# mushroomfire/mdapy

Hardware: AMD Instinct MI355X
Metric: atoms/sec for neighbor+CNA on 10M-atom FCC Cu; 1/2/4/8-GPU scaling (higher is better)
Workload: dtype f64 (CNA pair tests: f32 filter + f64 finish, labels exact); 1 GPU; FCC Cu a=3.615, 136^3 cells per GPU (10061824 atoms/GPU, 10061824 total), build_neighbor(rc=0.854a=3.08721, max_neigh=16) + fixed-cutoff CNA as one C-ABI call (mdh_build_neighbor_fcna: lists and labels), positions resident in HBM; atoms_per_gpu=10061824, max_neigh=16, parallelism=single, world_size_checked=1, launched_by=single process

## Files before the change

### mdapy_amd/csrc/cell_grid.hip

```cpp
#include "common.hpp"
#include "grid.hpp"
#include "assign_groups.hpp"
#include "grid_plan.hpp"
#include <algorithm>
#include <atomic>
#include <mutex>
#include <vector>

namespace mdh {
static std::atomic<int> g_indirect{[] { const char *e = std::getenv("MDH_INDIRECT"); return e ? std::atoi(e) : 1; }()};

struct CellPlanes { int p0, p1, p2, p3; int *bad; };
template <bool TRI, int K, bool SLOT = false>
__global__ __launch_bounds__(256) void k_assign(const double *__restrict__ x, const double *__restrict__ y,
                                                const double *__restrict__ z, int64_t N, DBox b, Grid g,
                                                int wrap_first, int2 *__restrict__ ent,
                                                unsigned *__restrict__ cell_count, unsigned *__restrict__ ctl, unsigned gen,
                                                double slack, unsigned short *__restrict__ mv, CellPlanes win,
                                                CellGrid::Packed *__restrict__ rec, int drop_absent, int *__restrict__ slots = nullptr,
                                                int2 *__restrict__ spill = nullptr, unsigned *__restrict__ spill_n = nullptr, int64_t slot_hi = 0)
{
    const int lane = threadIdx.x & 63;
    const int64_t i0 = ((int64_t)blockIdx.x * (blockDim.x >> 6) + (threadIdx.x >> 6)) * (64 * K) + lane;
    bool moved = false, outside = false, coded = false;
    double xr[K], yr[K], zr[K];
#pragma unroll
    for (int k = 0; k < K; ++k) {
        const int64_t i = i0 + 64 * k;
        xr[k] = yr[k] = zr[k] = 0.0;
        if (i < N) { xr[k] = x[i]; yr[k] = y[i]; zr[k] = z[i]; }
    }
    int cells[K];
#pragma unroll
    for (int k = 0; k < K; ++k) {
        const int64_t i = i0 + 64 * k;
        int cell = -1 - lane;
        const bool absent = drop_absent && i < N && xr[k] != xr[k];
// ... 54 lines not shown
#pragma unroll
    for (int k = 0; k < K; ++k) {
        const unsigned bs = __shfl(base[k], head[k], 64);
        const int64_t i = i0 + 64 * k;
        if (SLOT) {
            if (i < N && cells[k] >= 0) {
                const unsigned s = bs + (unsigned)slot[k];
                if (s < (unsigned)SLOT_CAP) slots[slot_pos(cells[k], (int)s, slot_hi)] = (int)i;
                else spill[atomicAdd(spill_n, 1u)] = make_int2(cells[k], (int)i);
            }
            continue;
        }
        if (i < N)
            ent[i] = make_int2(cells[k], (int)(bs + (unsigned)slot[k]));
    }
    if (__any(moved) && lane == 0)
        ctl[1] = gen;
    if (__any(coded) && lane == 0)
        ctl[2] = gen;
    if (__any(outside) && lane == 0)
        *win.bad = 1;
}

static constexpr int SCAN_BLOCK = 256;
static constexpr int SCAN_ITEMS = 4;
static constexpr int SCAN_ITEMS_BIG = 32;
static constexpr int64_t SCAN_BIG_FROM = 1 << 19;

__device__ __forceinline__ unsigned wave_incl_scan(unsigned v, int lane)
{
#pragma unroll
    for (int d = 1; d < 64; d <<= 1) {
        unsigned t = __shfl_up(v, d, 64);
        if (lane >= d) v += t;
// ... 193 lines not shown
    if (W == 4) {
        ce(0, 1); ce(2, 3); ce(0, 2); ce(1, 3); ce(1, 2);
    } else {
        ce(0, 1); ce(2, 3); ce(4, 5); ce(6, 7);
        ce(0, 2); ce(1, 3); ce(4, 6); ce(5, 7);
        ce(1, 2); ce(5, 6);
        ce(0, 4); ce(1, 5); ce(2, 6); ce(3, 7);
        ce(2, 4); ce(3, 5);
        ce(1, 2); ce(3, 4); ce(5, 6);
    }
#pragma unroll
    for (int u = 0; u < W; ++u)
        if (u < n) order[s + u] = id[u];
}

__device__ __forceinline__ void report_big_cell(unsigned *__restrict__ ctl, unsigned gen, int *__restrict__ sink, int n)
{
    if (__hip_atomic_load(&ctl[3], __ATOMIC_RELAXED, __HIP_MEMORY_SCOPE_AGENT) == gen)
        return;
    __hip_atomic_store(&ctl[3], gen, __ATOMIC_RELAXED, __HIP_MEMORY_SCOPE_AGENT);
    sink[1] = n;
}

__global__ __launch_bounds__(256) void k_sort_cells(const int *__restrict__ cell_start, int *__restrict__ order,
                                                    int64_t ncell, const int64_t *__restrict__ key, int *__restrict__ tmp,
                                                    unsigned *__restrict__ ctl = nullptr, unsigned gen = 0, int *__restrict__ big_sink = nullptr)
{
    int64_t c = (int64_t)blockIdx.x * blockDim.x + threadIdx.x;
    if (c >= ncell)
        return;
    const int s = cell_start[c], e = cell_start[c + 1];
    const int n = e - s;
    if (big_sink && n > SLOT_CAP) report_big_cell(ctl, gen, big_sink, n);
    if (n <= 1)
        return;
    if (n <= 4) {
        if (key) sort_cell_net<4, int64_t>(order, s, n, key);
        else sort_cell_net<4, int>(order, s, n, nullptr);
// ... 46 lines not shown
    if (staged) {
        for (int a = sub; a < n; a += 8) {
            const int mine = ids[lc * SORT_DENSE_CAP + a];
            int larger = 0;
            for (int q = 0; q < n; ++q) larger += ids[lc * SORT_DENSE_CAP + q] > mine ? 1 : 0;
            order[s + larger] = mine;
        }
    } else if (big) {
        for (int a = sub; a < n; a += 8) {
            const int mine = tmp[s + a];
            int larger = 0;
            for (int q = 0; q < n; ++q) larger += tmp[s + q] > mine ? 1 : 0;
            order[s + larger] = mine;
        }
    }
}

__global__ __launch_bounds__(256) void k_sort_slots(const unsigned *__restrict__ count, int *__restrict__ slots, int64_t ncell,
                                                    unsigned *__restrict__ idle, int64_t idle_n, unsigned *__restrict__ ctl, unsigned gen,
                                                    int *__restrict__ big_sink, int *__restrict__ flags, int64_t slot_hi)
{
    const int64_t c = (int64_t)blockIdx.x * blockDim.x + threadIdx.x;
    if (c == 0) {
        flags[0] = ctl[1] == gen ? 1 : 0; flags[1] = 0; flags[2] = 0; flags[3] = 0;
        flags[4] = ctl[2] == gen ? 1 : 0; flags[5] = 0; flags[6] = 0; flags[7] = 0;
    }
    if (c < idle_n) idle[c] = 0u;
    if (c >= ncell)
        return;
    const int full = (int)count[c];
    if (full > SLOT_CAP) report_big_cell(ctl, gen, big_sink, full);
    const int n = min(full, SLOT_CAP);
    if (n <= 1)
        return;
    int4 *cell = reinterpret_cast<int4 *>(slots + 4 * c), *cell_hi = reinterpret_cast<int4 *>(slots + slot_hi + 4 * c);
    auto ce = [](int &a, int &b) { const int hi = max(a, b), lo = min(a, b); a = hi; b = lo; };
    int4 q0 = cell[0];
    int id[8] = {q0.x, n > 1 ? q0.y : INT32_MIN, n > 2 ? q0.z : INT32_MIN, n > 3 ? q0.w : INT32_MIN, INT32_MIN, INT32_MIN, INT32_MIN, INT32_MIN};
    if (SLOT_CAP == 4 || n <= 4) {
        ce(id[0], id[1]); ce(id[2], id[3]); ce(id[0], id[2]); ce(id[1], id[3]); ce(id[1], id[2]);
        cell[0] = make_int4(id[0], id[1], id[2], id[3]);
        return;
    }
    const int4 q1 = cell_hi[0];
    id[4] = q1.x; id[5] = n > 5 ? q1.y : INT32_MIN; id[6] = n > 6 ? q1.z : INT32_MIN; id[7] = n > 7 ? q1.w : INT32_MIN;
    ce(id[0], id[1]); ce(id[2], id[3]); ce(id[4], id[5]); ce(id[6], id[7]);
    ce(id[0], id[2]); ce(id[1], id[3]); ce(id[4], id[6]); ce(id[5], id[7]);
    ce(id[1], id[2]); ce(id[5], id[6]);
    ce(id[0], id[4]); ce(id[1], id[5]); ce(id[2], id[6]); ce(id[3], id[7]);
    ce(id[2], id[4]); ce(id[3], id[5]);
    ce(id[1], id[2]); ce(id[3], id[4]); ce(id[5], id[6]);
    cell[0] = make_int4(id[0], id[1], id[2], id[3]);
    cell_hi[0] = make_int4(id[4], id[5], id[6], id[7]);
}

__global__ __launch_bounds__(256) void k_gather(const double *__restrict__ x, const double *__restrict__ y,
                                                const double *__restrict__ z, const int *__restrict__ order,
                                                double *__restrict__ xs, double *__restrict__ ys,
                                                double *__restrict__ zs, int64_t N,
                                                const unsigned short *__restrict__ mv, unsigned short *__restrict__ mvs,
                                                CellGrid::Packed *__restrict__ pk, const int *__restrict__ any_code,
                                                const int *__restrict__ n_binned)
{
    int64_t p = (int64_t)blockIdx.x * blockDim.x + threadIdx.x;
    if (p >= N)
        return;
    if (n_binned && p >= *n_binned)
        return;
// ... 251 lines not shown
    const size_t N = (size_t)bd.N;
    if (bd.slot()) {
        bd.slot_block = static_cast<unsigned *>(sc.alloc_kept(2 * sizeof(unsigned) * (size_t)(g.ncell + 128), Scope::KEEP_SLOT));
        if (bd.slot_block) {
            const size_t half = sc.held_bytes(bd.slot_block) / 8;
            bd.sb = slot_block_state(bd.slot_block);
            bd.cell_count = bd.slot_block + (size_t)bd.sb->next * half + 64;
            bd.slot_idle = bd.slot_block + (size_t)(1 - bd.sb->next) * half;
            bd.slot_idle_n = std::min<int64_t>(bd.sb->dirty[1 - bd.sb->next], (int64_t)half);
        }
        cg.slot_hi = 4 * g.ncell;
    } else {
        bd.cell_count = static_cast<unsigned *>(sc.alloc_kept(sizeof(unsigned) * (size_t)g.ncell, Scope::KEEP_ZERO));
    }
    bd.ctl = static_cast<unsigned *>(sc.alloc_kept(scan_ctl_bytes(g.ncell), Scope::KEEP_SCAN));
    cg.flags = sc.alloc_n<int>(8);
    cg.cell_start = bd.slot() ? reinterpret_cast<int *>(bd.cell_count) : sc.alloc_n<int>((size_t)g.ncell + 1);
    bd.ent = sc.alloc_n<int2>(N);
    cg.order = sc.alloc_n<int>(bd.slot() ? (size_t)g.ncell * SLOT_CAP + 4 : N + 4);
    bd.mv = sc.alloc_n<unsigned short>(N);
    switch (bd.pl.form) {
    case GridPlan::ARRAYS:
        cg.xs = sc.alloc_n<double>(N);
        cg.ys = sc.alloc_n<double>(N);
        cg.zs = sc.alloc_n<double>(N);
        cg.mvs = sc.alloc_n<unsigned short>(N);
        break;
    case GridPlan::RECORDS_GATHERED: cg.pk = sc.alloc_n<CellGrid::Packed>(N); break;
    case GridPlan::RECORDS_MOVED: cg.pk = sc.alloc_n<CellGrid::Packed>(N); bd.rec = sc.alloc_n<CellGrid::Packed>(N); break;
    case GridPlan::INDIRECT: case GridPlan::SLOT: break;
    }
// ... 9 lines not shown
    for (int d = 0; d < 3; ++d) nb[d] = std::max(1.0, std::floor(bd.b.thick[d] / edge));
    hipLaunchKernelGGL(k_order_far_flag, dim3(1), dim3(1024), 0, bd.st, bd.x, bd.y, bd.z, bd.N, bd.b, nb[0], nb[1], nb[2], word);
}

template <bool TRI, int K, bool SLOT>
static void launch_assign(const GridBuild &bd, const CellGrid &cg)
{
    const Grid &g = cg.g;
    const double slack = 0.01 / (g.rc_inv > 0 ? g.rc_inv : 1.0);
    const CellPlanes win{bd.pl.p0, bd.pl.p1, bd.pl.p2, bd.pl.p3, bd.bad};
    int2 *const ent = SLOT ? nullptr : bd.ent, *const spill = SLOT ? bd.ent : nullptr;
    int *const slots = SLOT ? cg.order : nullptr;
    unsigned *const spill_n = SLOT ? bd.cell_count - 64 : nullptr;
    hipLaunchKernelGGL((k_assign<TRI, K, SLOT>), dim3(grid_for(bd.N, 256 * K)), dim3(256), 0, bd.st, bd.x, bd.y, bd.z, bd.N, bd.b, g, (int)bd.rq.wrap_first,
                       ent, bd.cell_count, bd.ctl, bd.gen, slack, bd.mv, win, bd.rec, bd.pl.form != GridPlan::ARRAYS ? 1 : 0, slots, spill, spill_n,
                       SLOT ? cg.slot_hi : (int64_t)0);
}
static void bin_atoms(const GridBuild &bd, const CellGrid &cg)
{
    switch ((bd.b.tri ? 4 : 0) | (bd.pl.assign4 ? 2 : 0) | (bd.slot() ? 1 : 0)) {
    case 0: launch_assign<false, 1, false>(bd, cg); break;
    case 1: launch_assign<false, 1, true>(bd, cg); break;
    case 2: launch_assign<false, 4, false>(bd, cg); break;
    case 3: launch_assign<false, 4, true>(bd, cg); break;
    case 4: launch_assign<true, 1, false>(bd, cg); break;
    case 5: launch_assign<true, 1, true>(bd, cg); break;
    case 6: launch_assign<true, 4, false>(bd, cg); break;
    case 7: launch_assign<true, 4, true>(bd, cg); break;
    }
}

static int finish_slot_grid(Scope &sc, const GridBuild &bd, CellGrid &cg)
{
    const Grid &g = cg.g;
    hipLaunchKernelGGL(k_sort_slots, dim3(grid_for(std::max<int64_t>(g.ncell, bd.slot_idle_n), 256)), dim3(256), 0, bd.st, bd.cell_count, cg.order, g.ncell,
                       bd.slot_idle, bd.slot_idle_n, bd.ctl, bd.gen, bd.hist, cg.flags, cg.slot_hi);
    MDH_HIP(hipGetLastError());
    {
        std::lock_guard<std::mutex> lk(g_slot_mu);
        SlotBlock *sb = bd.sb;
        sb->dirty[1 - sb->next] = 0;
        sb->dirty[sb->next] = g.ncell + 64;
        sb->next = 1 - sb->next;
    }
    sc.keep_confirm(bd.slot_block);
    cg.big_stamp = bd.ctl + 3; cg.big_gen = bd.gen; cg.big_sink = bd.hist;
    cg.slot_cap = SLOT_CAP;
    cg.spill = bd.ent;
    cg.n_spill = bd.cell_count - 64;
    cg.ix = bd.x; cg.iy = bd.y; cg.iz = bd.z; cg.imv = bd.mv;
    return MDH_OK;
// ... 200 lines not shown
```

### mdapy_amd/csrc/grid.hpp

```cpp
#pragma once
#include "common.hpp"
#include "grid_plan.hpp"
#include <atomic>
#include <cmath>

namespace mdh {

struct Grid {
    int nc[3];
    int64_t ncell;
    double rc_inv;
    int mode;
};

namespace img {
constexpr int MAX_M = 14;
constexpr int ATOM_NEUTRAL = 15 | (15 << 5) | (15 << 10);
constexpr int CELL_NEUTRAL = 1 | (1 << 2) | (1 << 4);
constexpr int NEUTRAL = 16 | (16 << 5) | (16 << 10);
__host__ __device__ __forceinline__ int combine(int cc, int ca)
{
    return ((cc & 3) + (ca & 31)) | ((((cc >> 2) & 3) + ((ca >> 5) & 31)) << 5) | ((((cc >> 4) & 3) + ((ca >> 10) & 31)) << 10);
}
__host__ __device__ __forceinline__ int axis(int code, int d) { return ((code >> (5 * d)) & 31) - 16; }
// ... 8 lines not shown
    mutable bool flags_fresh = false;
    int *cell_start = nullptr;
    int *order = nullptr;
    double *xs = nullptr, *ys = nullptr, *zs = nullptr;
    int *flags = nullptr;
    unsigned short *mvs = nullptr;
    struct Packed { double x, y, z; int id, code; };
    Packed *pk = nullptr;
    const double *ix = nullptr, *iy = nullptr, *iz = nullptr;
    const unsigned short *imv = nullptr;
    int slot_cap = 0;
    int64_t slot_hi = 0;
    const int2 *spill = nullptr;
    const unsigned *n_spill = nullptr;
    int64_t n_binned = 0;
    const unsigned *big_stamp = nullptr;
    unsigned big_gen = 0;
    int *big_sink = nullptr;
};
__host__ __device__ __forceinline__ int64_t slot_pos(int64_t c, int k, int64_t hi) { return c * 4 + k + (k >= 4 ? hi - 4 : 0); }
struct SlotSpill { const int2 *list = nullptr; const unsigned *n = nullptr; int64_t hi = 0; };
struct SortedView {
    const double *xs, *ys, *zs;
    const int *order;
    const CellGrid::Packed *pk;
    bool indirect;
    __device__ __forceinline__ void get(int64_t q, double &x, double &y, double &z, int &id) const
    {
        if (pk) { const CellGrid::Packed r = pk[q]; x = r.x; y = r.y; z = r.z; id = r.id; }
        else if (indirect) { id = order[q]; x = xs[id]; y = ys[id]; z = zs[id]; }
        else { x = xs[q]; y = ys[q]; z = zs[q]; id = order[q]; }
    }
    __device__ __forceinline__ void get4(const int64_t (&q)[4], double (&x)[4], double (&y)[4], double (&z)[4], int (&id)[4]) const
    {
        if (pk) {
#pragma unroll
// ... 156 lines not shown
            for (int bb = c1 - 1; bb <= c1 + 1; ++bb) {
                const int64_t base = ((int64_t)ca * g.nc[1] + pmod(bb, g.nc[1])) * g.nc[2];
                for (int seg = 0; seg < (zrun ? 1 : 3); ++seg) {
                    const int64_t cell = base + (zrun ? c2 - 1 : pmod(c2 - 1 + seg, g.nc[2]));
                    if (SLOT) {
                        f(CellPiece{cell, cell_start[cell]});
                    } else {
                        const int s = cell_start[cell];
                        f(CellPiece{s, cell_start[cell + (zrun ? 3 : 1)] - s});
                    }
                }
            }
        }
    }
    __device__ __forceinline__ bool overflowed(const CellPiece &pc) const { return SLOT && pc.n > SLOT_CAP; }
    __device__ __forceinline__ int64_t pos(const CellPiece &pc, int k) const { return SLOT ? slot_pos(pc.at, k, sp.hi) : pc.at + k; }
    __device__ __forceinline__ int next_id_below(int64_t cell, int prev) const
    {
        int best = -1;
        for (int u = 0; u < SLOT_CAP; ++u) {
            const int v = sv.order[slot_pos(cell, u, sp.hi)];
            if (v < prev && v > best) best = v;
        }
        const unsigned ns = *sp.n;
        for (unsigned w = 0; w < ns; ++w) {
            const int2 e = sp.list[w];
            if ((int64_t)e.x == cell && e.y < prev && e.y > best) best = e.y;
        }
        return best;
    }
    template <class F>
// ... 50 lines not shown
```

### mdapy_amd/csrc/neighbor.hip

```cpp
#include "common.hpp"
#include "grid.hpp"
#include "cna_core.hpp"
#include <algorithm>

namespace mdh {

static int *g_moved_probe = nullptr;
int g_neighbor_variant = 0;

template <bool TRI, int MODE>
struct Centre {
    const DBox &b;
    int i;
    double xi, yi, zi, rcsq;
    int *__restrict__ verlet;
    double *__restrict__ dist;
    int64_t row, M;

    __device__ __forceinline__ Centre(const DBox &b_, int i_, double x, double y, double z, double rc, int *v, double *d, int64_t M_)
        : b(b_), i(i_), xi(x), yi(y), zi(z), rcsq(rc * rc), verlet(v), dist(d), row((int64_t)i_ * M_), M(M_) {}
    __device__ __forceinline__ bool hit(int j, double xq, double yq, double zq, double &d2) const
    {
        double dx = xq - xi, dy = yq - yi, dz = zq - zi;
        pbc<TRI>(b, dx, dy, dz);
// ... 11 lines not shown
    {
        if (lane == 0) nn[i] = cnt;
        if (MODE == 2) {
            const double pad = rc + 1.0;
            for (int64_t n = cnt + lane; n < M; n += stride) {
                verlet[row + n] = -1;
                dist[row + n] = pad;
            }
        }
    }
};

template <bool TRI, int MODE, bool SLOT>
__device__ __forceinline__ int overflowed_cell(const CellView<SLOT> &cv, const Centre<TRI, MODE> &c, int64_t cell, int cnt, bool store)
{
    for (int j = cv.next_id_below(cell, 0x7fffffff); j >= 0; j = cv.next_id_below(cell, j)) {
        double d2;
        if (!c.hit(j, cv.sv.xs[j], cv.sv.ys[j], cv.sv.zs[j], d2))
            continue;
        if (store) c.store(cnt, j, d2);
        ++cnt;
    }
    return cnt;
}

template <bool TRI, int MODE, bool SLOT>
__device__ __forceinline__ int neighbor_one(const CellView<SLOT> &cv, const Grid &g, const Centre<TRI, MODE> &c, double rc,
                                            int *__restrict__ nn, int c0, int c1, int c2)
{
    int cnt = 0;
    cv.for_each_piece(g, c0, c1, c2, [&](const CellPiece &pc) {
        if (cv.overflowed(pc)) {
            cnt = overflowed_cell(cv, c, pc.at, cnt, true);
            return;
        }
        for (int k0 = 0; k0 < pc.n; k0 += 4) {
            double xq[4], yq[4], zq[4], d2;
            int jq[4];
            int64_t q[4];
#pragma unroll
            for (int u = 0; u < 4; ++u) q[u] = cv.pos(pc, min(k0 + u, pc.n - 1));
            cv.sv.get4(q, xq, yq, zq, jq);
#pragma unroll
            for (int u = 0; u < 4; ++u)
                if (k0 + u < pc.n && c.hit(jq[u], xq[u], yq[u], zq[u], d2)) c.store(cnt++, jq[u], d2);
        }
    });
    c.finish(nn, rc, cnt, 0, 1);
    return cnt;
}

template <bool TRI, int MODE, bool SLOT>
__device__ __forceinline__ int neighbor_one_wave(const CellView<SLOT> &cv, const Grid &g, const Centre<TRI, MODE> &c, double rc,
                                                 int *__restrict__ nn, int c0, int c1, int c2)
{
    const int lane = (int)(threadIdx.x & 63);
    int cnt = 0;
    cv.for_each_piece(g, c0, c1, c2, [&](const CellPiece &pc) {
        if (cv.overflowed(pc)) {
            cnt = overflowed_cell(cv, c, pc.at, cnt, lane == 0);
            return;
        }
        for (int k0 = 0; k0 < pc.n; k0 += 64) {
            const int k = k0 + lane;
            bool hit = false;
            int j = -1;
            double d2 = 0.0;
            if (k < pc.n) {
                double xq, yq, zq;
                cv.sv.get(cv.pos(pc, k), xq, yq, zq, j);
                hit = c.hit(j, xq, yq, zq, d2);
            }
            const unsigned long long m = __ballot(hit);
            if (hit) c.store(cnt + __popcll(m & ((1ull << lane) - 1ull)), j, d2);
            cnt += __popcll(m);
        }
    });
    c.finish(nn, rc, cnt, lane, 64);
    return cnt;
}

template <bool TRI, int MODE, bool SLOT>
__device__ __forceinline__ void neighbor_atoms_body(const CellView<SLOT> &cv, int64_t N, const DBox &b, const Grid &g,
                                                  double rc, int *__restrict__ verlet, double *__restrict__ dist,
                                                  int *__restrict__ nn, int64_t M, int *__restrict__ max_count,
// ... 20 lines not shown
            }
        }
        if (mine) {
            cnt = max(cnt, neighbor_one(cv, g, Centre<TRI, MODE>(b, i, xi, yi, zi, rc, verlet, dist, M), rc, nn, c0, c1, c2));
            if (tf.cna_todo) defer(tf.cna_todo, i);
        }
    }
    if (MODE == 0) raise_max(max_count, wave_max(cnt));
}

template <bool TRI, int MODE, bool SLOT>
__global__ __launch_bounds__(256) void k_neighbor(SortedView sv, const int *__restrict__ cell_start, int64_t N, DBox b, Grid g, double rc,
                                                  int *__restrict__ verlet, double *__restrict__ dist, int *__restrict__ nn, int64_t M,
                                                  int *__restrict__ max_count, TileFilter tf, SlotSpill sp)
{
    if (tf.big_sink && blockIdx.x == 0 && threadIdx.x == 0)
        *tf.big_sink = *tf.big_stamp == tf.big_gen ? 1 : 0;
    neighbor_atoms_body<TRI, MODE>(CellView<SLOT>{sv, cell_start, sp}, N, b, g, rc, verlet, dist, nn, M, max_count, tf);
}

template <bool TRI, int MODE, bool SLOT>
__device__ __forceinline__ void neighbor_tiles_body(const CellView<SLOT> &cv, const DBox &b, const Grid &g, double rc,
                                                        int *__restrict__ verlet, double *__restrict__ dist, int *__restrict__ nn,
                                                        int64_t M, int *__restrict__ max_count, const TileFilter &tf)
{
    if (tf.moved && *tf.moved != 0)
        return;
    const int nlist = min(*tf.any, tf.list_cap);
    int best = 0;
    const int ncol = tf.tile * tf.tile;
    const int wave = (int)(threadIdx.x >> 6), nwave = (int)(blockDim.x >> 6);
// ... 38 lines not shown
{
    if (tf.listed_sink && blockIdx.x == 0 && threadIdx.x == 0)
        *tf.listed_sink = min(*tf.any, tf.list_cap);
    if (tf.big_sink && blockIdx.x == 0 && threadIdx.x == 0)
        *tf.big_sink = *tf.big_stamp == tf.big_gen ? 1 : 0;
    const CellView<SLOT> cv{sv, cell_start, sp};
    if (tf.moved && *tf.moved != 0) neighbor_atoms_body<TRI, MODE>(cv, N, b, g, rc, verlet, dist, nn, M, max_count, tf);
    else neighbor_tiles_body<TRI, MODE>(cv, b, g, rc, verlet, dist, nn, M, max_count, tf);
}

template <int MODE>
static void launch_neighbor(hipStream_t st, const CellGrid &cg, int64_t N, const DBox &b, double rc, int *verlet,
                            double *dist, int *nn, int64_t M, int *max_count, TileFilter tf = TileFilter{})
{
    dim3 grid(std::min(grid_for(N, 256), tf.list ? 2048 : 8192)), block(256);
    const SlotSpill sp{cg.spill, cg.n_spill, cg.slot_hi};
#define MDH_MOP(KERNEL, TRI, SLOT, ...) hipLaunchKernelGGL((KERNEL<TRI, MODE, SLOT>), grid, block, 0, st, view_of(cg), cg.cell_start, __VA_ARGS__, b, cg.g, rc, verlet, dist, nn, M, max_count, tf, sp)
    if (tf.list) {
        if (cg.slot_cap) { if (b.tri) MDH_MOP(k_neighbor_mop, true, true, N); else MDH_MOP(k_neighbor_mop, false, true, N); }
        else { if (b.tri) MDH_MOP(k_neighbor_mop, true, false, N); else MDH_MOP(k_neighbor_mop, false, false, N); }
        return;
    }
    if (cg.slot_cap) { if (b.tri) MDH_MOP(k_neighbor, true, true, N); else MDH_MOP(k_neighbor, false, true, N); }
    else { if (b.tri) MDH_MOP(k_neighbor, true, false, N); else MDH_MOP(k_neighbor, false, false, N); }
#undef MDH_MOP
}

__global__ __launch_bounds__(256) void k_max_i32(const int *__restrict__ v, int64_t n, int *__restrict__ out)
{
    int m = 0;
    for (int64_t i = (int64_t)blockIdx.x * blockDim.x + threadIdx.x; i < n; i += (int64_t)gridDim.x * blockDim.x) m = max(m, v[i]);
// ... 281 lines not shown
```

### mdapy_amd/csrc/neighbor_lane.hip

```cpp
#include "common.hpp"
#include "grid.hpp"
#include "cna_core.hpp"
#include <algorithm>
#include <cmath>
#include <type_traits>
#include <cstdio>
#include <cstdlib>
#include <cstring>

namespace mdh {
namespace lane {

constexpr int NW = 4;
constexpr int CEN_CAP = 80 * NW;
__host__ __device__ constexpr int ticket_row(int M, bool cna_rows) { return (cna_rows && ((M + 4) & ~3) < 28) ? 28 : ((M + 4) & ~3); }
static constexpr int NEUTRAL = img::CELL_NEUTRAL;
static constexpr int NEUTRAL3 = img::NEUTRAL;

struct FastDiv {
    unsigned mul, sh1, sh2, d;
    __device__ __forceinline__ unsigned div(unsigned n) const
    {
        const unsigned t = __umulhi(mul, n);
        return (t + ((n - t) >> sh1)) >> sh2;
// ... 231 lines not shown
            const int y = __builtin_amdgcn_mov_dpp(x, 0xB1, 0xF, 0xF, true);
            P[pp + 1][w] = bit_select(odd1, P[pp + 1][w], y);
            P[pp][w] = bit_select(odd1, y, P[pp][w]);
        }
#pragma unroll
    for (int pp = 0; pp < 2; ++pp)
#pragma unroll
        for (int w = 0; w < 4; ++w) {
            const int x = bit_select(odd2, P[pp][w], P[pp + 2][w]);
            const int y = __builtin_amdgcn_mov_dpp(x, 0x4E, 0xF, 0xF, true);
            P[pp + 2][w] = bit_select(odd2, P[pp + 2][w], y);
            P[pp][w] = bit_select(odd2, y, P[pp][w]);
        }
}

struct IndirectSrc { const double *x, *y, *z; const unsigned short *mv; const int *order; };
__device__ __forceinline__ CellGrid::Packed load_atom(const IndirectSrc &src, int id, int coded)
{
    int code = (int)img::ATOM_NEUTRAL;
    if (coded) code = src.mv[id];
    return CellGrid::Packed{src.x[id], src.y[id], src.z[id], id, code};
}
struct __attribute__((packed, aligned(4))) Ids4 { int v[4]; };
template <bool IND>
__device__ __forceinline__ CellGrid::Packed load_record(const CellGrid::Packed *__restrict__ pk, const IndirectSrc &src, int q, int coded)
{
    if (!IND)
        return pk[q];
    return load_atom(src, src.order[q], coded);
}

// ... 54 lines not shown
            t2 = t.id - (int)col * nt2;
            t0 = (int)ts.by_nt1.div(col);
            t1 = (int)col - t0 * nt1;
        }
        t.T0 = t0 * TXY; t.T1 = t1 * TXY; t.T2 = t2 * TZ;
        t.empty = t.T2 >= g.nc[2];
        return t;
    };
    auto halo_of = [&](const Tile &t) {
        Halo h{0, 0, NEUTRAL, 0, false, false};
        if (tid < NH && !t.empty) {
            const int hcol = (int)(((unsigned)tid * ts.mhz) >> 16);
            h.hz = tid - hcol * HZ;
            const int hx = (int)(((unsigned)hcol * ts.mhxy) >> 16), hy = hcol - hx * HXY;
            const int g0 = t.T0 + hx - 1, g1 = t.T1 + hy - 1, g2 = t.T2 + h.hz - 1;
            const bool in0 = b.pbc[0] ? (g0 >= -1 && g0 <= g.nc[0]) : (g0 >= 0 && g0 < g.nc[0]);
            const bool in1 = b.pbc[1] ? (g1 >= -1 && g1 <= g.nc[1]) : (g1 >= 0 && g1 < g.nc[1]);
            const bool in2 = b.pbc[2] ? (g2 >= -1 && g2 <= g.nc[2]) : (g2 >= 0 && g2 < g.nc[2]);
            if (in0 && in1 && in2) {
                bool over = false;
                const int a0 = g0 < 0 ? g0 + g.nc[0] : (g0 >= g.nc[0] ? g0 - g.nc[0] : g0);
                const int a1 = g1 < 0 ? g1 + g.nc[1] : (g1 >= g.nc[1] ? g1 - g.nc[1] : g1);
                const int a2 = g2 < 0 ? g2 + g.nc[2] : (g2 >= g.nc[2] ? g2 - g.nc[2] : g2);
                const int c = (a0 * g.nc[1] + a1) * g.nc[2] + a2;
                if (SLOT) {
                    const int n = cell_start[c];
                    h.src = c << 2;
                    h.cnt = min(n, SLOT_CAP);
                    over = n > SLOT_CAP;
                } else {
                    h.src = cell_start[c];
                    h.cnt = cell_start[c + 1] - h.src;
                }
                const int n0 = g0 < 0 ? 1 : (g0 >= g.nc[0] ? -1 : 0);
                const int n1 = g1 < 0 ? 1 : (g1 >= g.nc[1] ? -1 : 0);
                const int n2 = g2 < 0 ? 1 : (g2 >= g.nc[2] ? -1 : 0);
                h.img = (n0 + 1) | ((n1 + 1) << 2) | ((n2 + 1) << 4);
                if (SLOT && over) h.img |= 64;
                h.edge = (!b.pbc[0] && (a0 == 0 || a0 == g.nc[0] - 1)) || (!b.pbc[1] && (a1 == 0 || a1 == g.nc[1] - 1)) ||
                         (!b.pbc[2] && (a2 == 0 || a2 == g.nc[2] - 1));
                h.centre = hx >= 1 && hx <= TXY && hy >= 1 && hy <= TXY && h.hz >= 1 && h.hz <= TZ && g0 < g.nc[0] && g1 < g.nc[1] && g2 < g.nc[2] &&
                           g0 >= cen_lo && g0 < cen_hi;
            }
        }
        return h;
    };
    auto request = [&](const Halo &h, double (&ra)[4], double (&rb)[4], double (&rc4)[4], int (&rd)[4], int (&rm)[4]) {
        Ids4 ids{};
        if (IND) ids = *reinterpret_cast<const Ids4 *>(isrc.order + h.src);
#pragma unroll
        for (int v = 0; v < 4; ++v) {
            const int q = h.cnt > 0 ? h.src + min(v, h.cnt - 1) : 0;
            const CellGrid::Packed a = IND ? load_atom(isrc, v < h.cnt ? ids.v[v] : (h.cnt > 0 ? ids.v[0] : 0), coded) : load_record<false>(pk, isrc, q, coded);
            ra[v] = a.x; rb[v] = a.y; rc4[v] = a.z; rd[v] = a.id; rm[v] = a.code;
        }
    };
    for (int jt = jt0 + (int)(blockIdx.x >> 3); jt < per; jt += (int)(gridDim.x >> 3)) {
        const int slot = (int)(blockIdx.x & 7) * per + jt;
        if (slot >= nlive)
            break;
        const Tile tile = tile_of(slot);
        STAMP(0);
        Halo cur = halo_of(tile);
#ifdef MDH_STAMPS
        asm volatile("" : "+v"(cur.src), "+v"(cur.cnt));
        STAMP(1);
#endif
        double pa[4], pb[4], pc[4];
// ... 67 lines not shown
                            uy = (float)((bb[v] - b.h[4] * (double)img::axis(code, 1)) - Y0);
                            uz = (float)((c[v] - b.h[8] * (double)img::axis(code, 2)) - Z0);
                            general = true;
                        }
                        if (!TRI && edge)
                            far = far || !(ux >= flo && ux <= fhx && uy >= flo && uy <= fhx && uz >= flo && uz <= fhz);
                        const int p = off0 + k + v;
                        f4[p] = make_float4(ux, uy, uz, __int_as_float(d[v]));
                        lxy[p] = make_double2(a[v], bb[v]);
                        lz[p] = c[v];
                        lsh[p] = (unsigned short)code;
                        if (centre_cell) cen[coff + k + v] = (unsigned)p | ((unsigned)tid << 11);
                    }
                }
            };
            if (TK8) {
                for (int k = 0; k < cnt; k += 4) {
                    double a[4], bb[4], c[4];
                    int d[4], m[4];
#pragma unroll
                    for (int v = 0; v < 4; ++v) {
                        if (k == 0) { a[v] = pa[v]; bb[v] = pb[v]; c[v] = pc[v]; d[v] = pd[v]; m[v] = pm[v]; }
                        else {
                            const int kv = min(k + v, cnt - 1);
                            const int q = src + kv + (SLOT && kv >= 4 ? slot_hi : 0);
                            const CellGrid::Packed r = load_record<IND>(pk, isrc, q, coded);
                            a[v] = r.x; bb[v] = r.y; c[v] = r.z; d[v] = r.id; m[v] = r.code;
                        }
                    }
                    stage4(k, a, bb, c, d, m);
                }
            } else {
                double a[4], bb[4], c[4];
                int d[4], m[4];
#pragma unroll
                for (int v = 0; v < 4; ++v) { a[v] = pa[v]; bb[v] = pb[v]; c[v] = pc[v]; d[v] = pd[v]; m[v] = pm[v]; }
                for (int k = 0; k < cnt; k += 4) {
                    double na[4], nb[4], nc[4];
                    int nd[4], nm[4];
#pragma unroll
                    for (int v = 0; v < 4; ++v) {
                        const int kv = min(k + 4 + v, cnt - 1);
                        const int q = src + kv + (SLOT && kv >= 4 ? slot_hi : 0);
                        const CellGrid::Packed r = load_record<IND>(pk, isrc, q, coded);
                        na[v] = r.x; nb[v] = r.y; nc[v] = r.z; nd[v] = r.id; nm[v] = r.code;
                    }
                    stage4(k, a, bb, c, d, m);
#pragma unroll
                    for (int v = 0; v < 4; ++v) { a[v] = na[v]; bb[v] = nb[v]; c[v] = nc[v]; d[v] = nd[v]; m[v] = nm[v]; }
                }
            }
            if (general) s_flag[0] = 1;
            if (far) s_flag[1] = 1;
        }
        __syncthreads();
        STAMP(3);
        if (ok && (s_flag[1] | s_flag[2]))
            ok = false;
// ... 644 lines not shown
        hipLaunchKernelGGL(k_tile_compact, dim3(grid_for(ntiles, 256)), dim3(256), 0, st, live, slot, (int)ntiles, tile_list);
        const int64_t est_live = std::max<int64_t>(1, plan.occupied / std::max(1, ts.txy * ts.txy * ts.tz) * 2);
        per = std::max(1, std::min(per, (int)((est_live + est_live / 4 + 7) / 8)));
        list_mode = 1;
    }
    const dim3 grid((unsigned)(per * 8));
    const size_t lds = lds_bytes(plan.cap, count ? 1 : M, plan.tk8, plan.rw, pattern != nullptr);
    const int cen_lo = cg.cen_hi > cg.cen_lo ? cg.cen_lo : 0, cen_hi = cg.cen_hi > cg.cen_lo ? cg.cen_hi : 0x7fffffff;
    const int Mi = (int)M, wp = fill_pads ? (rows.ids_only ? 3 : 1) : 0;
    const float negc = -plan.mid;
    const int nt2b = nt[2] * nsub;
    const bool slice_pass = plan.last_listed != 0;
    const dim3 grid2(1024u);
    const Shape ts2 = make_shape(ts.txy, 1, nt[1], nt2b);
    const bool indirect = !cg.pk;
    const lane::IndirectSrc isrc{cg.ix, cg.iy, cg.iz, cg.imv, cg.order};
    const int slot_hi = cg.slot_cap ? (int)(cg.slot_hi - 4) : 0;
#define MDH_LANE_PASS_I(COUNT, TRI, LOOP, FCNA, TK8, IND, SLOT, GRID, JT0, ...)                                                                 \
    do {                                                                                                                                  \
        if (lds > 60 * 1024)                             \
            (void)hipFuncSetAttribute(reinterpret_cast<const void *>(&k_neighbor_lane<COUNT, TRI, LOOP, FCNA, TK8, IND, SLOT>), hipFuncAttributeMaxDynamicSharedMemorySize, (int)lds); \
        hipLaunchKernelGGL((k_neighbor_lane<COUNT, TRI, LOOP, FCNA, TK8, IND, SLOT>), GRID, dim3(NW * 64), lds, st, cg.pk, cg.cell_start, b, \
                           cg.g, rc, negc, plan.T, verlet, dist, nn, Mi, wp, plan.cap, cg.flags, nullptr, __VA_ARGS__, pattern, tf.cna_todo, JT0, plan.rw, tile_base, plan.listed_sink, \
                           cen_lo, cen_hi, isrc, slot_hi); \
    } while (0)
#define MDH_LANE_PASS(COUNT, TRI, LOOP, FCNA, TK8, GRID, JT0, ...)                                                                        \
    do {                                                                                                                                  \
        if (indirect && cg.slot_cap) MDH_LANE_PASS_I(COUNT, TRI, LOOP, FCNA, TK8, true, true, GRID, JT0, __VA_ARGS__);                    \
        else if (indirect) MDH_LANE_PASS_I(COUNT, TRI, LOOP, FCNA, TK8, true, false, GRID, JT0, __VA_ARGS__);                             \
        else MDH_LANE_PASS_I(COUNT, TRI, LOOP, FCNA, TK8, false, false, GRID, JT0, __VA_ARGS__);                                          \
    } while (0)
// ... 58 lines not shown
```

Before: 7.651 billion atoms/s.

## Drop slot-sort kernel; sort cell slots on the fly in neighbor consumers

Removes the separate k_sort_slots launch. The idle-buffer zeroing and the flag setting move into k_assign, and the per-cell sorting network moves into the neighbor kernels, which sort the slot ids in registers when they load them. Big-cell reporting is moved into the consumers as well. The halo setup also gains a fast path for interior tiles that skips the boundary wrap arithmetic. This saves one kernel launch and a full pass over the slot array, at the cost of repeating the sort each time a cell is read (27 neighbours) and adding flag-protocol complexity.

New measurement: 7.709 billion atoms/s, median of 6. No clear change (+0.8%).

```diff
diff --git a/mdapy_amd/csrc/cell_grid.hip b/mdapy_amd/csrc/cell_grid.hip
--- a/mdapy_amd/csrc/cell_grid.hip
+++ b/mdapy_amd/csrc/cell_grid.hip
@@ -18,9 +18,17 @@
                                                 unsigned *__restrict__ cell_count, unsigned *__restrict__ ctl, unsigned gen,
                                                 double slack, unsigned short *__restrict__ mv, CellPlanes win,
                                                 CellGrid::Packed *__restrict__ rec, int drop_absent, int *__restrict__ slots = nullptr,
-                                                int2 *__restrict__ spill = nullptr, unsigned *__restrict__ spill_n = nullptr, int64_t slot_hi = 0)
+                                                int2 *__restrict__ spill = nullptr, unsigned *__restrict__ spill_n = nullptr, int64_t slot_hi = 0,
+                                                unsigned *__restrict__ idle = nullptr, int64_t idle_n = 0)
 {
     const int lane = threadIdx.x & 63;
+    if (SLOT) {
+        const int64_t stride = 4 * (int64_t)gridDim.x * blockDim.x;
+        for (int64_t w = 4 * ((int64_t)blockIdx.x * blockDim.x + threadIdx.x); w < idle_n; w += stride) {
+            if (w + 4 <= idle_n) *reinterpret_cast<uint4 *>(idle + w) = make_uint4(0u, 0u, 0u, 0u);
+            else for (int64_t t = w; t < idle_n; ++t) idle[t] = 0u;
+        }
+    }
     const int64_t i0 = ((int64_t)blockIdx.x * (blockDim.x >> 6) + (threadIdx.x >> 6)) * (64 * K) + lane;
     bool moved = false, outside = false, coded = false;
     double xr[K], yr[K], zr[K];
@@ -105,10 +113,14 @@
         if (i < N)
             ent[i] = make_int2(cells[k], (int)(bs + (unsigned)slot[k]));
     }
-    if (__any(moved) && lane == 0)
+    if (__any(moved) && lane == 0) {
         ctl[1] = gen;
-    if (__any(coded) && lane == 0)
+        if (SLOT) spill_n[8] = 1u;
+    }
+    if (__any(coded) && lane == 0) {
         ctl[2] = gen;
+        if (SLOT) spill_n[8 + 4] = 1u;
+    }
     if (__any(outside) && lane == 0)
         *win.bad = 1;
 }
@@ -332,14 +344,6 @@
         if (u < n) order[s + u] = id[u];
 }
 
-__device__ __forceinline__ void report_big_cell(unsigned *__restrict__ ctl, unsigned gen, int *__restrict__ sink, int n)
-{
-    if (__hip_atomic_load(&ctl[3], __ATOMIC_RELAXED, __HIP_MEMORY_SCOPE_AGENT) == gen)
-        return;
-    __hip_atomic_store(&ctl[3], gen, __ATOMIC_RELAXED, __HIP_MEMORY_SCOPE_AGENT);
-    sink[1] = n;
-}
-
 __global__ __launch_bounds__(256) void k_sort_cells(const int *__restrict__ cell_start, int *__restrict__ order,
                                                     int64_t ncell, const int64_t *__restrict__ key, int *__restrict__ tmp,
                                                     unsigned *__restrict__ ctl = nullptr, unsigned gen = 0, int *__restrict__ big_sink = nullptr)
@@ -416,44 +420,6 @@
             order[s + larger] = mine;
         }
     }
-}
-
-__global__ __launch_bounds__(256) void k_sort_slots(const unsigned *__restrict__ count, int *__restrict__ slots, int64_t ncell,
-                                                    unsigned *__restrict__ idle, int64_t idle_n, unsigned *__restrict__ ctl, unsigned gen,
-                                                    int *__restrict__ big_sink, int *__restrict__ flags, int64_t slot_hi)
-{
-    const int64_t c = (int64_t)blockIdx.x * blockDim.x + threadIdx.x;
-    if (c == 0) {
-        flags[0] = ctl[1] == gen ? 1 : 0; flags[1] = 0; flags[2] = 0; flags[3] = 0;
-        flags[4] = ctl[2] == gen ? 1 : 0; flags[5] = 0; flags[6] = 0; flags[7] = 0;
-    }
-    if (c < idle_n) idle[c] = 0u;
-    if (c >= ncell)
-        return;
-    const int full = (int)count[c];
-    if (full > SLOT_CAP) report_big_cell(ctl, gen, big_sink, full);
-    const int n = min(full, SLOT_CAP);
-    if (n <= 1)
-        return;
-    int4 *cell = reinterpret_cast<int4 *>(slots + 4 * c), *cell_hi = reinterpret_cast<int4 *>(slots + slot_hi + 4 * c);
-    auto ce = [](int &a, int &b) { const int hi = max(a, b), lo = min(a, b); a = hi; b = lo; };
-    int4 q0 = cell[0];
-    int id[8] = {q0.x, n > 1 ? q0.y : INT32_MIN, n > 2 ? q0.z : INT32_MIN, n > 3 ? q0.w : INT32_MIN, INT32_MIN, INT32_MIN, INT32_MIN, INT32_MIN};
-    if (SLOT_CAP == 4 || n <= 4) {
-        ce(id[0], id[1]); ce(id[2], id[3]); ce(id[0], id[2]); ce(id[1], id[3]); ce(id[1], id[2]);
-        cell[0] = make_int4(id[0], id[1], id[2], id[3]);
-        return;
-    }
-    const int4 q1 = cell_hi[0];
-    id[4] = q1.x; id[5] = n > 5 ? q1.y : INT32_MIN; id[6] = n > 6 ? q1.z : INT32_MIN; id[7] = n > 7 ? q1.w : INT32_MIN;
-    ce(id[0], id[1]); ce(id[2], id[3]); ce(id[4], id[5]); ce(id[6], id[7]);
-    ce(id[0], id[2]); ce(id[1], id[3]); ce(id[4], id[6]); ce(id[5], id[7]);
-    ce(id[1], id[2]); ce(id[5], id[6]);
-    ce(id[0], id[4]); ce(id[1], id[5]); ce(id[2], id[6]); ce(id[3], id[7]);
-    ce(id[2], id[4]); ce(id[3], id[5]);
-    ce(id[1], id[2]); ce(id[3], id[4]); ce(id[5], id[6]);
-    cell[0] = make_int4(id[0], id[1], id[2], id[3]);
-    cell_hi[0] = make_int4(id[4], id[5], id[6], id[7]);
 }
 
 __global__ __launch_bounds__(256) void k_gather(const double *__restrict__ x, const double *__restrict__ y,
@@ -735,7 +701,7 @@
         bd.cell_count = static_cast<unsigned *>(sc.alloc_kept(sizeof(unsigned) * (size_t)g.ncell, Scope::KEEP_ZERO));
     }
     bd.ctl = static_cast<unsigned *>(sc.alloc_kept(scan_ctl_bytes(g.ncell), Scope::KEEP_SCAN));
-    cg.flags = sc.alloc_n<int>(8);
+    cg.flags = bd.slot() ? (bd.slot_block ? reinterpret_cast<int *>(bd.cell_count - 64 + 8) : nullptr) : sc.alloc_n<int>(8);
     cg.cell_start = bd.slot() ? reinterpret_cast<int *>(bd.cell_count) : sc.alloc_n<int>((size_t)g.ncell + 1);
     bd.ent = sc.alloc_n<int2>(N);
     cg.order = sc.alloc_n<int>(bd.slot() ? (size_t)g.ncell * SLOT_CAP + 4 : N + 4);
@@ -775,7 +741,7 @@
     unsigned *const spill_n = SLOT ? bd.cell_count - 64 : nullptr;
     hipLaunchKernelGGL((k_assign<TRI, K, SLOT>), dim3(grid_for(bd.N, 256 * K)), dim3(256), 0, bd.st, bd.x, bd.y, bd.z, bd.N, bd.b, g, (int)bd.rq.wrap_first,
                        ent, bd.cell_count, bd.ctl, bd.gen, slack, bd.mv, win, bd.rec, bd.pl.form != GridPlan::ARRAYS ? 1 : 0, slots, spill, spill_n,
-                       SLOT ? cg.slot_hi : (int64_t)0);
+                       SLOT ? cg.slot_hi : (int64_t)0, SLOT ? bd.slot_idle : nullptr, SLOT ? bd.slot_idle_n : (int64_t)0);
 }
 static void bin_atoms(const GridBuild &bd, const CellGrid &cg)
 {
@@ -794,8 +760,6 @@
 static int finish_slot_grid(Scope &sc, const GridBuild &bd, CellGrid &cg)
 {
     const Grid &g = cg.g;
-    hipLaunchKernelGGL(k_sort_slots, dim3(grid_for(std::max<int64_t>(g.ncell, bd.slot_idle_n), 256)), dim3(256), 0, bd.st, bd.cell_count, cg.order, g.ncell,
-                       bd.slot_idle, bd.slot_idle_n, bd.ctl, bd.gen, bd.hist, cg.flags, cg.slot_hi);
     MDH_HIP(hipGetLastError());
     {
         std::lock_guard<std::mutex> lk(g_slot_mu);
diff --git a/mdapy_amd/csrc/grid.hpp b/mdapy_amd/csrc/grid.hpp
--- a/mdapy_amd/csrc/grid.hpp
+++ b/mdapy_amd/csrc/grid.hpp
@@ -46,12 +46,34 @@
     const int2 *spill = nullptr;
     const unsigned *n_spill = nullptr;
     int64_t n_binned = 0;
-    const unsigned *big_stamp = nullptr;
+    unsigned *big_stamp = nullptr;
     unsigned big_gen = 0;
     int *big_sink = nullptr;
 };
+__device__ __forceinline__ bool report_big_cell(unsigned *__restrict__ ctl, unsigned gen, int *__restrict__ sink, int n)
+{
+    if (__hip_atomic_load(&ctl[3], __ATOMIC_RELAXED, __HIP_MEMORY_SCOPE_AGENT) == gen)
+        return false;
+    __hip_atomic_store(&ctl[3], gen, __ATOMIC_RELAXED, __HIP_MEMORY_SCOPE_AGENT);
+    sink[1] = n;
+    return true;
+}
 __host__ __device__ __forceinline__ int64_t slot_pos(int64_t c, int k, int64_t hi) { return c * 4 + k + (k >= 4 ? hi - 4 : 0); }
-struct SlotSpill { const int2 *list = nullptr; const unsigned *n = nullptr; int64_t hi = 0; };
+__device__ __forceinline__ void slot_ce(int &a, int &b) { const int hi = max(a, b), lo = min(a, b); a = hi; b = lo; }
+__device__ __forceinline__ void sort_slots4(int (&id)[4])
+{
+    slot_ce(id[0], id[1]); slot_ce(id[2], id[3]); slot_ce(id[0], id[2]); slot_ce(id[1], id[3]); slot_ce(id[1], id[2]);
+}
+__device__ __forceinline__ void sort_slots8(int (&id)[8])
+{
+    slot_ce(id[0], id[1]); slot_ce(id[2], id[3]); slot_ce(id[4], id[5]); slot_ce(id[6], id[7]);
+    slot_ce(id[0], id[2]); slot_ce(id[1], id[3]); slot_ce(id[4], id[6]); slot_ce(id[5], id[7]);
+    slot_ce(id[1], id[2]); slot_ce(id[5], id[6]);
+    slot_ce(id[0], id[4]); slot_ce(id[1], id[5]); slot_ce(id[2], id[6]); slot_ce(id[3], id[7]);
+    slot_ce(id[2], id[4]); slot_ce(id[3], id[5]);
+    slot_ce(id[1], id[2]); slot_ce(id[3], id[4]); slot_ce(id[5], id[6]);
+}
+struct SlotSpill { const int2 *list = nullptr; const unsigned *n = nullptr; int64_t hi = 0; unsigned *big_ctl = nullptr; unsigned big_gen = 0; int *big_sink = nullptr; };
 struct SortedView {
     const double *xs, *ys, *zs;
     const int *order;
@@ -238,7 +260,22 @@
         }
     }
     __device__ __forceinline__ bool overflowed(const CellPiece &pc) const { return SLOT && pc.n > SLOT_CAP; }
-    __device__ __forceinline__ int64_t pos(const CellPiece &pc, int k) const { return SLOT ? slot_pos(pc.at, k, sp.hi) : pc.at + k; }
+    __device__ __forceinline__ int64_t pos(const CellPiece &pc, int k) const { return pc.at + k; }
+    __device__ __forceinline__ void slot_ids(const CellPiece &pc, int (&id)[SLOT_CAP]) const
+    {
+        const int4 lo = *reinterpret_cast<const int4 *>(sv.order + 4 * pc.at);
+        id[0] = pc.n > 0 ? lo.x : INT32_MIN; id[1] = pc.n > 1 ? lo.y : INT32_MIN; id[2] = pc.n > 2 ? lo.z : INT32_MIN; id[3] = pc.n > 3 ? lo.w : INT32_MIN;
+        id[4] = id[5] = id[6] = id[7] = INT32_MIN;
+        if (pc.n <= 4) {
+            int q[4] = {id[0], id[1], id[2], id[3]};
+            sort_slots4(q);
+            id[0] = q[0]; id[1] = q[1]; id[2] = q[2]; id[3] = q[3];
+            return;
+        }
+        const int4 up = *reinterpret_cast<const int4 *>(sv.order + sp.hi + 4 * pc.at);
+        id[4] = up.x; id[5] = pc.n > 5 ? up.y : INT32_MIN; id[6] = pc.n > 6 ? up.z : INT32_MIN; id[7] = pc.n > 7 ? up.w : INT32_MIN;
+        sort_slots8(id);
+    }
     __device__ __forceinline__ int next_id_below(int64_t cell, int prev) const
     {
         int best = -1;
diff --git a/mdapy_amd/csrc/neighbor.hip b/mdapy_amd/csrc/neighbor.hip
--- a/mdapy_amd/csrc/neighbor.hip
+++ b/mdapy_amd/csrc/neighbor.hip
@@ -49,6 +49,7 @@
 template <bool TRI, int MODE, bool SLOT>
 __device__ __forceinline__ int overflowed_cell(const CellView<SLOT> &cv, const Centre<TRI, MODE> &c, int64_t cell, int cnt, bool store)
 {
+    if (cv.sp.big_sink && report_big_cell(cv.sp.big_ctl, cv.sp.big_gen, cv.sp.big_sink, cv.cell_start[cell])) cv.sp.big_sink[0] = 1;
     for (int j = cv.next_id_below(cell, 0x7fffffff); j >= 0; j = cv.next_id_below(cell, j)) {
         double d2;
         if (!c.hit(j, cv.sv.xs[j], cv.sv.ys[j], cv.sv.zs[j], d2))
@@ -69,6 +70,27 @@
             cnt = overflowed_cell(cv, c, pc.at, cnt, true);
             return;
         }
+        if constexpr (SLOT) {
+            if (pc.n <= 0)
+                return;
+            int id[SLOT_CAP];
+            cv.slot_ids(pc, id);
+#pragma unroll
+            for (int k0 = 0; k0 < SLOT_CAP; k0 += 4) {
+                if (k0 >= pc.n)
+                    break;
+                double xq[4], yq[4], zq[4], d2;
+                int jq[4];
+#pragma unroll
+                for (int u = 0; u < 4; ++u) jq[u] = k0 + u < pc.n ? id[k0 + u] : id[0];
+#pragma unroll
+                for (int u = 0; u < 4; ++u) { xq[u] = cv.sv.xs[jq[u]]; yq[u] = cv.sv.ys[jq[u]]; zq[u] = cv.sv.zs[jq[u]]; }
+#pragma unroll
+                for (int u = 0; u < 4; ++u)
+                    if (k0 + u < pc.n && c.hit(jq[u], xq[u], yq[u], zq[u], d2)) c.store(cnt++, jq[u], d2);
+            }
+            return;
+        }
         for (int k0 = 0; k0 < pc.n; k0 += 4) {
             double xq[4], yq[4], zq[4], d2;
             int jq[4];
@@ -96,6 +118,8 @@
             cnt = overflowed_cell(cv, c, pc.at, cnt, lane == 0);
             return;
         }
+        int id[SLOT_CAP];
+        if constexpr (SLOT) { if (pc.n > 0) cv.slot_ids(pc, id); }
         for (int k0 = 0; k0 < pc.n; k0 += 64) {
             const int k = k0 + lane;
             bool hit = false;
@@ -103,7 +127,14 @@
             double d2 = 0.0;
             if (k < pc.n) {
                 double xq, yq, zq;
-                cv.sv.get(cv.pos(pc, k), xq, yq, zq, j);
+                if constexpr (SLOT) {
+                    j = id[0];
+#pragma unroll
+                    for (int u = 1; u < SLOT_CAP; ++u) j = k == u ? id[u] : j;
+                    xq = cv.sv.xs[j]; yq = cv.sv.ys[j]; zq = cv.sv.zs[j];
+                } else {
+                    cv.sv.get(cv.pos(pc, k), xq, yq, zq, j);
+                }
                 hit = c.hit(j, xq, yq, zq, d2);
             }
             const unsigned long long m = __ballot(hit);
@@ -154,7 +185,7 @@
                                                   int *__restrict__ verlet, double *__restrict__ dist, int *__restrict__ nn, int64_t M,
                                                   int *__restrict__ max_count, TileFilter tf, SlotSpill sp)
 {
-    if (tf.big_sink && blockIdx.x == 0 && threadIdx.x == 0)
+    if (tf.big_sink && !sp.big_sink && blockIdx.x == 0 && threadIdx.x == 0)
         *tf.big_sink = *tf.big_stamp == tf.big_gen ? 1 : 0;
     neighbor_atoms_body<TRI, MODE>(CellView<SLOT>{sv, cell_start, sp}, N, b, g, rc, verlet, dist, nn, M, max_count, tf);
 }
@@ -223,7 +254,8 @@
                             double *dist, int *nn, int64_t M, int *max_count, TileFilter tf = TileFilter{})
 {
     dim3 grid(std::min(grid_for(N, 256), tf.list ? 2048 : 8192)), block(256);
-    const SlotSpill sp{cg.spill, cg.n_spill, cg.slot_hi};
+    SlotSpill sp{cg.spill, cg.n_spill, cg.slot_hi};
+    if (cg.slot_cap && !tf.list && cg.big_sink) { sp.big_ctl = cg.big_stamp - 3; sp.big_gen = cg.big_gen; sp.big_sink = cg.big_sink; }
 #define MDH_MOP(KERNEL, TRI, SLOT, ...) hipLaunchKernelGGL((KERNEL<TRI, MODE, SLOT>), grid, block, 0, st, view_of(cg), cg.cell_start, __VA_ARGS__, b, cg.g, rc, verlet, dist, nn, M, max_count, tf, sp)
     if (tf.list) {
         if (cg.slot_cap) { if (b.tri) MDH_MOP(k_neighbor_mop, true, true, N); else MDH_MOP(k_neighbor_mop, false, true, N); }
diff --git a/mdapy_amd/csrc/neighbor_lane.hip b/mdapy_amd/csrc/neighbor_lane.hip
--- a/mdapy_amd/csrc/neighbor_lane.hip
+++ b/mdapy_amd/csrc/neighbor_lane.hip
@@ -269,7 +269,7 @@
         }
 }
 
-struct IndirectSrc { const double *x, *y, *z; const unsigned short *mv; const int *order; };
+struct IndirectSrc { const double *x, *y, *z; const unsigned short *mv; const int *order; unsigned *big_ctl; unsigned big_gen; int *big_sink; };
 __device__ __forceinline__ CellGrid::Packed load_atom(const IndirectSrc &src, int id, int coded)
 {
     int code = (int)img::ATOM_NEUTRAL;
@@ -354,33 +354,44 @@
             h.hz = tid - hcol * HZ;
             const int hx = (int)(((unsigned)hcol * ts.mhxy) >> 16), hy = hcol - hx * HXY;
             const int g0 = t.T0 + hx - 1, g1 = t.T1 + hy - 1, g2 = t.T2 + h.hz - 1;
-            const bool in0 = b.pbc[0] ? (g0 >= -1 && g0 <= g.nc[0]) : (g0 >= 0 && g0 < g.nc[0]);
-            const bool in1 = b.pbc[1] ? (g1 >= -1 && g1 <= g.nc[1]) : (g1 >= 0 && g1 < g.nc[1]);
-            const bool in2 = b.pbc[2] ? (g2 >= -1 && g2 <= g.nc[2]) : (g2 >= 0 && g2 < g.nc[2]);
-            if (in0 && in1 && in2) {
+            const bool interior = t.T0 >= (b.pbc[0] ? 1 : 2) && t.T0 + TXY <= g.nc[0] - (b.pbc[0] ? 1 : 2) &&
+                                  t.T1 >= (b.pbc[1] ? 1 : 2) && t.T1 + TXY <= g.nc[1] - (b.pbc[1] ? 1 : 2) &&
+                                  t.T2 >= (b.pbc[2] ? 1 : 2) && t.T2 + TZ <= g.nc[2] - (b.pbc[2] ? 1 : 2);
+            bool in = true, edge = false, in_grid = true;
+            int a0 = g0, a1 = g1, a2 = g2, im = NEUTRAL;
+            if (!interior) {
+                const bool in0 = b.pbc[0] ? (g0 >= -1 && g0 <= g.nc[0]) : (g0 >= 0 && g0 < g.nc[0]);
+                const bool in1 = b.pbc[1] ? (g1 >= -1 && g1 <= g.nc[1]) : (g1 >= 0 && g1 < g.nc[1]);
+                const bool in2 = b.pbc[2] ? (g2 >= -1 && g2 <= g.nc[2]) : (g2 >= 0 && g2 < g.nc[2]);
+                in = in0 && in1 && in2;
+                a0 = g0 < 0 ? g0 + g.nc[0] : (g0 >= g.nc[0] ? g0 - g.nc[0] : g0);
+                a1 = g1 < 0 ? g1 + g.nc[1] : (g1 >= g.nc[1] ? g1 - g.nc[1] : g1);
+                a2 = g2 < 0 ? g2 + g.nc[2] : (g2 >= g.nc[2] ? g2 - g.nc[2] : g2);
+                const int n0 = g0 < 0 ? 1 : (g0 >= g.nc[0] ? -1 : 0);
+                const int n1 = g1 < 0 ? 1 : (g1 >= g.nc[1] ? -1 : 0);
+                const int n2 = g2 < 0 ? 1 : (g2 >= g.nc[2] ? -1 : 0);
+                im = (n0 + 1) | ((n1 + 1) << 2) | ((n2 + 1) << 4);
+                edge = (!b.pbc[0] && (a0 == 0 || a0 == g.nc[0] - 1)) || (!b.pbc[1] && (a1 == 0 || a1 == g.nc[1] - 1)) ||
+                       (!b.pbc[2] && (a2 == 0 || a2 == g.nc[2] - 1));
+                in_grid = g0 < g.nc[0] && g1 < g.nc[1] && g2 < g.nc[2];
+            }
+            if (in) {
                 bool over = false;
-                const int a0 = g0 < 0 ? g0 + g.nc[0] : (g0 >= g.nc[0] ? g0 - g.nc[0] : g0);
-                const int a1 = g1 < 0 ? g1 + g.nc[1] : (g1 >= g.nc[1] ? g1 - g.nc[1] : g1);
-                const int a2 = g2 < 0 ? g2 + g.nc[2] : (g2 >= g.nc[2] ? g2 - g.nc[2] : g2);
                 const int c = (a0 * g.nc[1] + a1) * g.nc[2] + a2;
                 if (SLOT) {
                     const int n = cell_start[c];
                     h.src = c << 2;
                     h.cnt = min(n, SLOT_CAP);
                     over = n > SLOT_CAP;
+                    if (over && isrc.big_sink) report_big_cell(isrc.big_ctl, isrc.big_gen, isrc.big_sink, n);
                 } else {
                     h.src = cell_start[c];
                     h.cnt = cell_start[c + 1] - h.src;
                 }
-                const int n0 = g0 < 0 ? 1 : (g0 >= g.nc[0] ? -1 : 0);
-                const int n1 = g1 < 0 ? 1 : (g1 >= g.nc[1] ? -1 : 0);
-                const int n2 = g2 < 0 ? 1 : (g2 >= g.nc[2] ? -1 : 0);
-                h.img = (n0 + 1) | ((n1 + 1) << 2) | ((n2 + 1) << 4);
+                h.img = im;
                 if (SLOT && over) h.img |= 64;
-                h.edge = (!b.pbc[0] && (a0 == 0 || a0 == g.nc[0] - 1)) || (!b.pbc[1] && (a1 == 0 || a1 == g.nc[1] - 1)) ||
-                         (!b.pbc[2] && (a2 == 0 || a2 == g.nc[2] - 1));
-                h.centre = hx >= 1 && hx <= TXY && hy >= 1 && hy <= TXY && h.hz >= 1 && h.hz <= TZ && g0 < g.nc[0] && g1 < g.nc[1] && g2 < g.nc[2] &&
-                           g0 >= cen_lo && g0 < cen_hi;
+                h.edge = edge;
+                h.centre = hx >= 1 && hx <= TXY && hy >= 1 && hy <= TXY && h.hz >= 1 && h.hz <= TZ && in_grid && g0 >= cen_lo && g0 < cen_hi;
             }
         }
         return h;
@@ -388,10 +399,17 @@
     auto request = [&](const Halo &h, double (&ra)[4], double (&rb)[4], double (&rc4)[4], int (&rd)[4], int (&rm)[4]) {
         Ids4 ids{};
         if (IND) ids = *reinterpret_cast<const Ids4 *>(isrc.order + h.src);
+        if (SLOT) {
+            int sid[4] = {h.cnt > 0 ? ids.v[0] : INT32_MIN, h.cnt > 1 ? ids.v[1] : INT32_MIN, h.cnt > 2 ? ids.v[2] : INT32_MIN, h.cnt > 3 ? ids.v[3] : INT32_MIN};
+            sort_slots4(sid);
+#pragma unroll
+            for (int v = 0; v < 4; ++v) ids.v[v] = max(sid[v], 0);
+        }
 #pragma unroll
         for (int v = 0; v < 4; ++v) {
             const int q = h.cnt > 0 ? h.src + min(v, h.cnt - 1) : 0;
-            const CellGrid::Packed a = IND ? load_atom(isrc, v < h.cnt ? ids.v[v] : (h.cnt > 0 ? ids.v[0] : 0), coded) : load_record<false>(pk, isrc, q, coded);
+            const CellGrid::Packed a = SLOT ? load_atom(isrc, ids.v[v], coded)
+                                       : IND ? load_atom(isrc, v < h.cnt ? ids.v[v] : (h.cnt > 0 ? ids.v[0] : 0), coded) : load_record<false>(pk, isrc, q, coded);
             ra[v] = a.x; rb[v] = a.y; rc4[v] = a.z; rd[v] = a.id; rm[v] = a.code;
         }
     };
@@ -489,7 +507,26 @@
                     }
                 }
             };
-            if (TK8) {
+            if (SLOT) {
+                if (cnt <= 4) {
+                    stage4(0, pa, pb, pc, pd, pm);
+                } else {
+                    const Ids4 up = *reinterpret_cast<const Ids4 *>(isrc.order + src + 4 + slot_hi);
+                    int sid[8] = {pd[0], pd[1], pd[2], pd[3], up.v[0], cnt > 5 ? up.v[1] : INT32_MIN, cnt > 6 ? up.v[2] : INT32_MIN, cnt > 7 ? up.v[3] : INT32_MIN};
+                    sort_slots8(sid);
+#pragma unroll
+                    for (int half = 0; half < 2; ++half) {
+                        double a[4], bb[4], c[4];
+                        int d[4], m[4];
+#pragma unroll
+                        for (int v = 0; v < 4; ++v) {
+                            const CellGrid::Packed r = load_atom(isrc, 4 * half + v < cnt ? sid[4 * half + v] : sid[0], coded);
+                            a[v] = r.x; bb[v] = r.y; c[v] = r.z; d[v] = r.id; m[v] = r.code;
+                        }
+                        stage4(4 * half, a, bb, c, d, m);
+                    }
+                }
+            } else if (TK8) {
                 for (int k = 0; k < cnt; k += 4) {
                     double a[4], bb[4], c[4];
                     int d[4], m[4];
@@ -498,7 +535,7 @@
                         if (k == 0) { a[v] = pa[v]; bb[v] = pb[v]; c[v] = pc[v]; d[v] = pd[v]; m[v] = pm[v]; }
                         else {
                             const int kv = min(k + v, cnt - 1);
-                            const int q = src + kv + (SLOT && kv >= 4 ? slot_hi : 0);
+                            const int q = src + kv;
                             const CellGrid::Packed r = load_record<IND>(pk, isrc, q, coded);
                             a[v] = r.x; bb[v] = r.y; c[v] = r.z; d[v] = r.id; m[v] = r.code;
                         }
@@ -516,7 +553,7 @@
 #pragma unroll
                     for (int v = 0; v < 4; ++v) {
                         const int kv = min(k + 4 + v, cnt - 1);
-                        const int q = src + kv + (SLOT && kv >= 4 ? slot_hi : 0);
+                        const int q = src + kv;
                         const CellGrid::Packed r = load_record<IND>(pk, isrc, q, coded);
                         na[v] = r.x; nb[v] = r.y; nc[v] = r.z; nd[v] = r.id; nm[v] = r.code;
                     }
@@ -1191,7 +1228,7 @@
     const dim3 grid2(1024u);
     const Shape ts2 = make_shape(ts.txy, 1, nt[1], nt2b);
     const bool indirect = !cg.pk;
-    const lane::IndirectSrc isrc{cg.ix, cg.iy, cg.iz, cg.imv, cg.order};
+    const lane::IndirectSrc isrc{cg.ix, cg.iy, cg.iz, cg.imv, cg.order, cg.slot_cap && cg.big_sink ? cg.big_stamp - 3 : nullptr, cg.big_gen, cg.slot_cap ? cg.big_sink : nullptr};
     const int slot_hi = cg.slot_cap ? (int)(cg.slot_hi - 4) : 0;
 #define MDH_LANE_PASS_I(COUNT, TRI, LOOP, FCNA, TK8, IND, SLOT, GRID, JT0, ...)                                                                 \
     do {                                                                                                                                  \
```
